# l646773422/h264-lab

Hardware: AMD Instinct MI355X
Metric: 1080p macroblocks/sec (higher is better)
Workload: dtype u8

## Files before the change

### h264-lab_amd/csrc/enc_mb.h

```cpp
#ifndef H264E_ENC_MB_H
#define H264E_ENC_MB_H

#include <stddef.h>
#include "enc_kernels.h"

struct GCtx { mv32 mv_left[4], mv_tl[4], mv_top[8]; };
#define GSCR_OFF(t) ((t) == 0 ? 0 : (t) == 1 ? 1024 : (t) == 2 ? 1536 : 2048)
#define GSCR_BYTES 2304

struct MbBuf
{
    alignas(16) uint8_t inp[256];
    alignas(16) uint8_t inp_c[128];
    alignas(16) uint8_t pred[256];
    alignas(4) uint8_t pix_top[36];
    alignas(4) uint8_t ptop[96];
    mv32 mv_top[8];
    uint8_t nnz_top[8];
    int8_t i4_top[4];
    uint32_t df_nz_top;
    int top_type, top_qp;
    mv32 mv[16], mvd[16];
    int type, cost, used_cand;
    mv32 mv_skip_pred;
};

struct RowLds
{
    mv32 mv_left[4], mv_tl[4];
    uint8_t nnz_left[8];
    int8_t i4_left[4];
    alignas(4) uint8_t pix_left[32];
    uint8_t pix_tl[4];
    uint32_t df_nzflag;
    mv32 df_mv[25];
    int left_type, left_qp;
    alignas(4) uint8_t strip_y[16*4];
    alignas(4) uint8_t strip_c[2][8*4];
    alignas(4) uint8_t brec[64];
    BitW bw;
    int skip_run, lead_skips, coded_any;
    int far_reads[3];
    int far_fail[3];
    int16_t slice_row[H264E_MAX_SLICES + 2];
    unsigned long long prof[4][32], prof_last[4], prof_c0, prof_w0;
    int f_noskip, f_bound, f_inter, f_decided, f_wdone, f_stop;
    int early_bound;
    int f_t3req, f_t3done;
    int f_front, d_type[2];
    int t3_sad_best, t3_lim[4];
    mv32 t3_mv_best;

    MbBuf mb[2];
    alignas(4) uint8_t trec[72];

    int8_t i4_mode[16];
    alignas(4) uint8_t bs[32];
    I4Scratch i4s;
    uint8_t nzctx[12];
    alignas(16) uint8_t pred_c[128];
    alignas(16) uint8_t i16pred[256];
    alignas(16) uint8_t tt[256];
    alignas(16) uint8_t i4rec[17*24];
    alignas(16) uint8_t ytile[20*YT_STRIDE];
    alignas(16) uint8_t ctile[2][10*CT_STRIDE];
    alignas(16) qblk_t qy[16];
    qblk_t qu[4], qv[4];
    int16_t dcy[16], dcu[4], dcv[4], lev_dcy[16], lev_dcu[4], lev_dcv[4];

    CavlcTab cavlc;
    DfTab dftab;
    int qconst[6];
    uint16_t qdat[2][42];

    mv32 part_mv[4][4], part_mvd[4][4];
    GCtx gctx[4];
    int gcost[4], gnum[4];
    alignas(16) uint8_t win[WIN_W*WIN_STRIDE + 16];
    alignas(16) uint8_t skip_pred[256];
    alignas(16) uint8_t skip_pred_c[128];
    alignas(16) uint8_t gtest[4][256];
    alignas(16) uint8_t gscr[GSCR_BYTES];

};
#define ROWLDS_INTRA_BYTES offsetof(RowLds, part_mv)

struct MbCtx
{
    const h264e_geom_t *G;
    int speed, slice_type;
    mv32 clu[2];
    const mv32 *clu_per_mb;
    Plane ref[3];
    RefView rv;
    gu8 *dec[3];
    int x, y, num, avail, type, cost, i16_mode, cropped, used_cand;
    int slice_top;
    mv32 mv_skip_pred;
    unsigned nz_mask;
    int qp;
    int lambda_mv, lambda_q4, skip_thr, skip_thr_i4, lambda_i4, lambda_i16;
};

struct rect_t { int x0, y0, x1, y1; };

DEV int in_rect(mv32 v, const rect_t &r) { return mvy(v) >= r.y0 && mvy(v) <= r.y1 && mvx(v) >= r.x0 && mvx(v) <= r.x1; }
DEV mv32 clip_rect(mv32 v, const rect_t &r) { return mvmk(imin(imax(mvx(v), r.x0), r.x1), imin(imax(mvy(v), r.y0), r.y1)); }
DEV mv32 mb_abs(const MbCtx &m, mv32 v) { return mvadd(v, mvmk(m.x*64, m.y*64)); }
DEV int mv_cost(const MbCtx &m, mv32 v, mv32 pred)
{
    return MUL_LAMBDA(se_len(mvx(v) - mvx(pred)) + se_len(mvy(v) - mvy(pred)), m.lambda_mv);
}
DEV rect_t mv_limit(const MbCtx &m) { rect_t r = { m.G->lim_x0, m.G->lim_y0, m.G->lim_x1, m.G->lim_y1 }; return r; }
DEV rect_t mv_qlimit(const MbCtx &m) { rect_t r = { m.G->lim_x0 + 16, m.G->lim_y0 + 16, m.G->lim_x1 - 16, m.G->lim_y1 - 16 }; return r; }


DEV int med3(int a, int b, int c) { return imax(imin(imax(a, b), c), imin(a, b)); }

DEV void mvp_put_arr(mv32 *mv_left, mv32 *mv_tl, mv32 *mv_top, int x, int y, int w, int h, mv32 mv)
{
    mv_tl[y] = mv_top[x + w - 1];
    for (int i = 1; i < h; i++) mv_tl[y + i] = mv;
    for (int i = 0; i < h; i++) mv_left[y + i] = mv;
    for (int i = 0; i < w; i++) mv_top[x + i] = mv;
}
DEV void mvp_put(RowLds &L, MbBuf &B, int x, int y, int w, int h, mv32 mv) { mvp_put_arr(L.mv_left, L.mv_tl, B.mv_top, x, y, w, h, mv); }

DEV mv32 mvp_get_arr(const mv32 *mv_left, const mv32 *mv_tl, const mv32 *mv_top, int flag, int x, int y, int w, int h)
{
    int type = 1;
    mv32 a = mv_left[y], b = mv_top[x], c = mv_top[x + w], d = mv_tl[y], ret = 0;
// ... 821 lines not shown
```

### h264-lab_amd/csrc/enc_row.h

```cpp
#ifndef H264E_ENC_ROW_H
#define H264E_ENC_ROW_H

#include "enc_mb.h"

#define GEOM_WIDE 0
#define GEOM_NARROW 1
#define GEOM_INTRA 2

struct ChainG
{
    GLOBAL_AS h264e_mbbottom_t *bottom;
    GLOBAL_AS h264e_mbpend_t *pend;
    GLOBAL_AS int *progress;
    GLOBAL_AS uint32_t *rowbits;
    GLOBAL_AS h264e_rowmeta_t *rowmeta;
    GLOBAL_AS h264e_mbrec_t *mbrec;
    GLOBAL_AS uint8_t *arena;
    uint32_t arena_cap;
    GLOBAL_AS uint8_t *nal_arena;
    uint32_t nal_cap;
    GLOBAL_AS uint32_t *cursor;
    GLOBAL_AS h264e_frameout_t *fout;
    GLOBAL_AS int *far_reads;
    unsigned long long *prof;
};
DEV ChainG chain_view(const h264e_chain_dev_t &C)
{
    ChainG g;
    g.bottom = (GLOBAL_AS h264e_mbbottom_t *)C.bottom; g.pend = (GLOBAL_AS h264e_mbpend_t *)C.pend; g.progress = (GLOBAL_AS int *)C.progress;
    g.rowbits = (GLOBAL_AS uint32_t *)C.rowbits; g.rowmeta = (GLOBAL_AS h264e_rowmeta_t *)C.rowmeta;
    g.mbrec = (GLOBAL_AS h264e_mbrec_t *)C.mbrec; g.arena = (GLOBAL_AS uint8_t *)C.arena; g.arena_cap = C.arena_cap; g.nal_arena = (GLOBAL_AS uint8_t *)C.nal_arena; g.nal_cap = C.nal_cap;
    g.cursor = (GLOBAL_AS uint32_t *)C.cursor; g.fout = (GLOBAL_AS h264e_frameout_t *)C.fout; g.far_reads = (GLOBAL_AS int *)C.far_reads; g.prof = C.prof;
    return g;
}

DEV void row_begin(RowLds &L, const h264e_geom_t &G, const ChainG &C, const h264e_frame_task_t &T, int row)
{
    WAVE_FOR(l)
    {
        if (l < 4) { L.mv_left[l] = 0; L.mv_tl[l] = 0; L.i4_left[l] = -1; L.pix_tl[l] = 0; }
        if (l < 8) L.nnz_left[l] = NNZ_NA;
        if (l < 32) L.pix_left[l] = 0;
        if (l < 25) L.df_mv[l] = 0;
        L.strip_y[l] = 0;
        L.strip_c[l >> 5][l & 31] = 0;
    }
    L.df_nzflag = 0;
    L.left_type = 0;
    L.left_qp = T.qp;
    L.bw.acc = 0; L.bw.nacc = 0; L.bw.pos = 0; L.bw.overflow = 0;
    L.bw.cap = (uint32_t)G.row_words;
    L.bw.buf = C.rowbits + (size_t)row*G.row_words;
    L.skip_run = 0; L.lead_skips = 0; L.coded_any = 0; L.far_reads[0] = L.far_reads[1] = L.far_reads[2] = 0; L.far_fail[0] = L.far_fail[1] = L.far_fail[2] = 0;
    L.f_noskip = L.f_bound = L.f_inter = L.f_decided = L.f_wdone = L.f_stop = 0; L.early_bound = 0; L.f_t3req = L.f_t3done = L.f_front = 0;
    WAVE_FOR(l) { if (l <= H264E_MAX_SLICES) L.slice_row[l] = l <= T.nslices ? T.slice_row[l] : (int16_t)0x7fff; }
    WAVE_FOR(l)
    {
        for (int k = l; k < 84; k += 64) L.qdat[k/42][k%42] = T.qdat[k/42][k%42];
    }
    cavlc_tab_load(L.cavlc);
    df_tab_load(L.dftab);
    L.qconst[0] = k_lambda_mv_q4[T.qp]; L.qconst[1] = k_lambda_q4[T.qp]; L.qconst[2] = k_skip_thr_inter[T.qp];
    L.qconst[3] = k_skip_thr_i4x4[T.qp]; L.qconst[4] = k_lambda_i4_q4[T.qp]; L.qconst[5] = k_lambda_i16_q4[T.qp];
    for (int i = 0; i < 32; i++) L.prof[0][i] = L.prof[1][i] = L.prof[2][i] = L.prof[3][i] = 0;
    L.prof_last[0] = L.prof_last[1] = 0;
    PROF_ROW_BEGIN(L);
    wave_sync();
    PROF_ROW_SYNC(L);
}

#define LOAD_TOP_ALL 0
#define LOAD_TOP_MV 1
#define LOAD_TOP_REST 2
template <int PART> DEV void load_top(RowLds &L, MbBuf &B, const h264e_geom_t &G, const GLOBAL_AS h264e_mbbottom_t *above, const GLOBAL_AS h264e_mbpend_t *pend_above, int x, int have_top)
{
    if (PART == LOAD_TOP_MV)
    {
        WAVE_FOR(l)
        {
            if (l < 4) B.mv_top[l] = have_top ? (mv32)cload32((const gu8 *)(above + x) + 32 + 4*l) : 0;
            else if (l == 4) B.mv_top[4] = (have_top && x + 1 < G.nmbx) ? (mv32)cload32((const gu8 *)(above + x + 1) + 32) : 0;
        }
        wave_sync();
        return;
    }
    if (have_top)
    {
        WAVE_FOR(l)
        {
            if (l < 16) lds32_store(L.trec + 4*l, cload32((const gu8 *)(above + x) + 4*l));
            else if (l == 16) lds32_store(L.trec + 64, x + 1 < G.nmbx ? cload32((const gu8 *)(above + x + 1)) : 0u);
            else if (l == 17) lds32_store(L.trec + 68, x + 1 < G.nmbx ? cload32((const gu8 *)(above + x + 1) + 32) : 0u);
            else if (l >= 32 && l < 56) lds32_store(B.ptop + 4*(l - 32), cload32((const gu8 *)(pend_above + x) + 4*(l - 32)));
        }
        wave_sync();
        WAVE_FOR(l)
        {
            if (l < 8) lds32_store(B.pix_top + 4*l, lds32(L.trec + 4*l));
            else if (l < 12) { if (PART == LOAD_TOP_ALL) B.mv_top[l - 8] = (mv32)lds32(L.trec + 32 + 4*(l - 8)); }
            else if (l < 20) B.nnz_top[l - 12] = L.trec[48 + l - 12];
            else if (l < 24) B.i4_top[l - 20] = (int8_t)L.trec[56 + l - 20];
            else if (l == 24) { B.df_nz_top = L.trec[60]; B.top_type = (int8_t)L.trec[61]; B.top_qp = L.trec[62]; }
            else if (l == 25) lds32_store(B.pix_top + 32, lds32(L.trec + 64));
            else if (l == 26) { if (PART == LOAD_TOP_ALL) B.mv_top[4] = (mv32)lds32(L.trec + 68); }
        }
    } else
    {
        WAVE_FOR(l)
        {
            if (l < 36) B.pix_top[l] = 0;
            if (l < 5 && PART == LOAD_TOP_ALL) B.mv_top[l] = 0;
            if (l < 8) B.nnz_top[l] = NNZ_NA;
            if (l < 4) B.i4_top[l] = -1;
            if (l == 0) { B.df_nz_top = 0; B.top_type = 0; B.top_qp = 0; }
        }
    }
    wave_sync();
}

DEV void load_input(MbBuf &B, const h264e_geom_t &G, const RowTask &T, int mbx, int mby)
{
    const bool inside = (mbx + 1)*16 <= G.width && (mby + 1)*16 <= G.height;
    WAVE_FOR(l)
    {
        {
            int r = l >> 2, c = l & 3, yy = imin(mby*16 + r, G.height - 1);
            const gu8 *p = (const gu8 *)T.in[0] + (size_t)yy*T.in_stride[0];
            uint32_t v = 0;
            if (inside) v = gload32(p + mbx*16 + 4*c);
            else for (int k = 0; k < 4; k++) v |= (uint32_t)p[imin(mbx*16 + 4*c + k, G.width - 1)] << (8*k);
            lds32_store(B.inp + 16*r + 4*c, v);
        }
        if (l < 32)
        {
            int pl = l >> 4, r = (l >> 1) & 7, c = l & 1, yy = imin(mby*8 + r, G.height/2 - 1);
            const gu8 *p = (const gu8 *)(pl ? T.in[2] : T.in[1]) + (size_t)yy*(pl ? T.in_stride[2] : T.in_stride[1]);
            uint32_t v = 0;
            if (inside) v = gload32(p + mbx*8 + 4*c);
            else for (int k = 0; k < 4; k++) v |= (uint32_t)p[imin(mbx*8 + 4*c + k, G.width/2 - 1)] << (8*k);
            lds32_store(B.inp_c + 16*r + 8*pl + 4*c, v);
        }
    }
    wave_sync();
}

template <int GEOM> DEV void row_prefetch(RowLds &L, const h264e_geom_t &G, const RowTask &T, int row, int x)
{
    load_input(L.mb[x & 1], G, T, x, row);
    if (GEOM != GEOM_INTRA && T.slice_type == 0)
    {
        Plane P;
        P.p = (const gu8 *)T.ref[0]; P.w = G.W; P.h = G.H; P.stride = G.W;
        wave_load_window(L.win, P, x*16 - WIN_M, row*16 - WIN_M, T.narrow);
    }
}

template <int GEOM> DEV void mb_ctx_init(MbCtx &m, RowLds &L, const h264e_geom_t &G, const RowTask &T, int row, int x, int row0, int side)
{
    const bool have_top = row > row0;
    m.G = &G;
    m.speed = T.speed; m.slice_type = T.slice_type; m.clu[0] = T.clusters[0]; m.clu[1] = T.clusters[1]; m.clu_per_mb = T.clusters_per_mb;
    for (int c = 0; c < 3; c++)
    {
        m.ref[c].p = (const gu8 *)T.ref[c];
        m.ref[c].w = G.W >> (c ? 1 : 0); m.ref[c].h = G.H >> (c ? 1 : 0); m.ref[c].stride = m.ref[c].w;
        m.dec[c] = (gu8 *)T.dec[c];
    }
    m.x = x; m.y = row; m.num = row*G.nmbx + x;
    m.avail = (have_top ? AV_T : 0) | (have_top && x != G.nmbx - 1 ? AV_TR : 0) | (x > 0 ? AV_L : 0) | (have_top && x > 0 ? AV_TL : 0);
    m.slice_top = !have_top;
    m.cropped = G.cropping && ((x + 1)*16 > G.width || (row + 1)*16 > G.height);
    m.type = 0; m.cost = 0x7FFFFFFF; m.i16_mode = 0; m.used_cand = 0; m.mv_skip_pred = 0; m.nz_mask = 0;
    m.qp = T.qp;
    m.lambda_mv = uni(L.qconst[0]); m.lambda_q4 = uni(L.qconst[1]); m.skip_thr = uni(L.qconst[2]);
    m.skip_thr_i4 = uni(L.qconst[3]); m.lambda_i4 = uni(L.qconst[4]); m.lambda_i16 = uni(L.qconst[5]);
    m.rv.dep = (const GLOBAL_AS int *)T.dep_progress; m.rv.nmbx = G.nmbx; m.rv.nmby = G.nmby;
    m.rv.P = m.ref[0]; m.rv.win = (const lu8 *)L.win; m.rv.has_win = GEOM != GEOM_INTRA && T.slice_type == 0; m.rv.wx0 = x*16 - WIN_M; m.rv.wy0 = row*16 - WIN_M;
    m.rv.vw = GEOM == GEOM_NARROW ? H264E_NARROW_VW : WIN_W; m.rv.vh = GEOM == GEOM_NARROW ? H264E_NARROW_VH : WIN_W; m.rv.far = &L.far_reads[side]; m.rv.fail = &L.far_fail[side]; m.rv.slice_row = L.slice_row; m.rv.nslices = T.nslices; m.rv.spin_limit = G.spin_limit;
}

struct NoSignals { DEVM void noskip() const {} DEVM void bound(int) const {} DEVM bool helper() const { return false; } DEVM void t3_request(mv32, int, const rect_t &) const {} DEVM bool t3_wait() const { return true; } };
template <int GEOM, class SIG> DEV void mb_search(RowLds &L, MbBuf &B, const h264e_geom_t &G, const RowTask &T, int row, int x, int row0, SIG sig)
{
    MbCtx m;
    mb_ctx_init<GEOM>(m, L, G, T, row, x, row0, 0);
    STAMP(L, 1);
    if (GEOM != GEOM_INTRA && T.slice_type == 0) inter_choose(L, B, m, sig);
    STAMP(L, 7);
    B.type = m.type; B.cost = m.cost; B.used_cand = m.used_cand; B.mv_skip_pred = m.mv_skip_pred;
    wave_sync();
}

struct InterIsThere
{
    DEVM bool ready() const { return true; }
    DEVM bool wait_noskip_or_ready() const { return true; }
    DEVM bool wait_bound_or_ready() const { return true; }
    DEVM bool wait_ready() const { return true; }
    DEVM int early_bound() const { return 0x7fffffff; }
    DEVM bool before_decide() const { return true; }
};

template <class P> DEV bool mb_intra_decide(RowLds &L, MbBuf &B, MbCtx &m, const RowTask &T, P pol)
{
    bool have = pol.ready();
    if (!have)
    {
        if (!pol.wait_noskip_or_ready()) return false;
        have = pol.ready();
// ... 584 lines not shown
```

### h264-lab_amd/csrc/h264e_dev.h

```cpp
#ifndef H264E_DEV_H
#define H264E_DEV_H
#include <stdint.h>

#define H264E_MV_NA 0x8000
#define H264E_ORDER_PAD 0xffffffffu
#define H264E_MAX_SLICES 16
#define H264E_ROW_BYTES_PER_MB 2048

#define H264E_DEP_ROWS 2
#define H264E_DEP_COLS 3
#define H264E_FRAME_LAG (2*H264E_DEP_ROWS + H264E_DEP_COLS)
#define H264E_NARROW_VW 53
#define H264E_NARROW_VH 52
#define H264E_NARROW_DEP_ROWS 1
#define H264E_NARROW_DEP_COLS 2
#define H264E_NARROW_FRAME_LAG (2*H264E_NARROW_DEP_ROWS + H264E_NARROW_DEP_COLS)

typedef int32_t mv32;

typedef struct
{
    int width, height;
    int W, H;
    int nmbx, nmby, nmb, cropping;
    int lim_x0, lim_y0, lim_x1, lim_y1;
    int row_words;
    unsigned spin_limit;
    int test_stall_row;
    int fz_wait_all;
} h264e_geom_t;

typedef struct
{
    uint8_t pix[32];
    mv32 mv[4];
    uint8_t nnz[8];
    int8_t i4[4];
    uint8_t df_nz;
    int8_t type;
    uint8_t qp;
    uint8_t pad;
} h264e_mbbottom_t;

typedef struct
{
    uint8_t y[64];
    uint8_t c[2][16];
} h264e_mbpend_t;

typedef struct
{
    uint32_t nbits;
    int32_t lead_skips;
    int32_t trail_skips;
    int32_t overflow;
} h264e_rowmeta_t;

typedef struct
{
    mv32 mv0;
    int8_t type;
    uint8_t used_cand;
    uint8_t pad[2];
} h264e_mbrec_t;

typedef struct
{
    uint32_t offset;
    uint32_t nbytes;
    int32_t nslices;
    uint32_t slice_nbytes[H264E_MAX_SLICES];
    int32_t all_skipped;
    int32_t clusters_moved;
    int32_t overflow;
    int32_t far_reads;
    int32_t pad[2];
} h264e_frameout_t;

#define H264E_WALK_OK 1
#define H264E_WALK_BAD 2
#define H264E_WALK_VOID 3
typedef struct
// ... 84 lines not shown
```

### h264-lab_amd/csrc/h264e_kernels.hip

```cpp
#include <stdio.h>
#include <stdlib.h>
#include <string.h>
#include "enc_row.h"
#include "enc_selftest.h"
#include "../../include/h264e_hip.h"

#include <hip/hip_runtime.h>





#ifndef H264E_POLL_SLEEP
#define H264E_POLL_SLEEP 16
#endif
DEV int poll_progress(const GLOBAL_AS int *flag, int need, int &seen, unsigned spin_limit)
{
    unsigned spins = 0;
    for (;;)
    {
        seen = uni(__hip_atomic_load(flag, __ATOMIC_RELAXED, __HIP_MEMORY_SCOPE_AGENT));
        if (seen >= need) return 0;
        if (seen < 0) return seen;
        if (++spins > spin_limit) return -1;
// ... 236 lines not shown
                for (int k = 0; k < H264E_MAX_SLICES; k++) hd->slice_nbytes[k] = nal_bytes[k];
                hd->clusters_moved = F.clusters_moved; hd->overflow = F.overflow | exp_overflow; hd->far_reads = F.far_reads;
                hd->walk_status = wstatus; hd->first_bad = first_bad; hd->state_out[0] = ws[0]; hd->state_out[1] = ws[1];
                __builtin_amdgcn_fence(__ATOMIC_RELEASE, "");
                asm volatile("s_waitcnt vmcnt(0)" ::: "memory");
                __hip_atomic_store(&hd->done, T.launch_id, __ATOMIC_RELAXED, __HIP_MEMORY_SCOPE_SYSTEM);
            }
        }
        FZ_STAMP(36);
#ifdef H264E_STAMPS
        if (LANE == 0 && C.prof) atomicAdd(C.prof + 37, 1ull);
#endif
        return;
    }

    if (row < T.first_row) return;
    if (job == 0 && row == G.test_stall_row) return;
    if (wv == 0) row_begin(L, G, C, T, row);
    if (WAVES >= 2) __syncthreads();
    const RowTask RT = rowtask_load(T);
    int row0 = 0, row1 = G.nmby;
    for (int k = 0; k < T.nslices; k++)
        if (row >= T.slice_row[k] && row < T.slice_row[k + 1]) { row0 = T.slice_row[k]; row1 = T.slice_row[k + 1]; }
    row0 = uni(row0); row1 = uni(row1);
    GLOBAL_AS int *my_progress = C.progress + row;
    GLOBAL_AS unsigned long long *mb_counter = (GLOBAL_AS unsigned long long *)uniptr(T.mb_counter);
    const auto count_mbs = [&](int n) { if (mb_counter && n > 0 && LANE == 0) __hip_atomic_fetch_add(mb_counter, (unsigned long long)n, __ATOMIC_RELAXED, __HIP_MEMORY_SCOPE_AGENT); };

    if (WAVES == 1 || wv == 0)
    {
        const GLOBAL_AS int *abort_word = (const GLOBAL_AS int *)uniptr(T.abort_word);
        const int launch_id = uni(T.launch_id);
        int seen = 0, seen_dep = 0;
        constexpr bool NARROW = GEOM == GEOM_NARROW;
        constexpr int DEP_ROWS = NARROW ? H264E_NARROW_DEP_ROWS : H264E_DEP_ROWS, DEP_COLS = NARROW ? H264E_NARROW_DEP_COLS : H264E_DEP_COLS;
        unsigned long long deps = 0;
        int ndeps = 0;
        if (T.dep_progress)
        {
            const int lo = imax(row - 2, 0), hi = imin(row + DEP_ROWS, G.nmby - 1);
            deps = (unsigned long long)hi; ndeps = 1;
            for (int k = T.nslices - 1; k >= 1; k--)
            {
                const int last = T.slice_row[k] - 1;
                if (last >= lo && last < hi) { deps |= (unsigned long long)last << (10*ndeps); ndeps++; }
            }
            ndeps = uni(ndeps);
        }
        for (int x = 0; x < G.nmbx; x++)
        {
            const int need = row > row0 ? imin(x + 2, G.nmbx) : 0;
            const int need_dep = RT.dep_progress ? imin(x + DEP_COLS, G.nmbx) : 0;
            int st = 0;
            const int abort_v = abort_word ? __hip_atomic_load(abort_word, __ATOMIC_RELAXED, __HIP_MEMORY_SCOPE_AGENT) : launch_id - 1;
            const GLOBAL_AS int *above = C.progress + (WAVES >= 2 ? G.nmby : 0) + (row - 1);
            const int early = seen < need ? __hip_atomic_load(above, __ATOMIC_RELAXED, __HIP_MEMORY_SCOPE_AGENT) : seen;
            if (seen_dep < need_dep)
            {
                int lowest = 0x7fffffff;
                for (int k = 0; k < ndeps && !st; k++)
                {
                    int sk = 0;
                    st = poll_progress((const GLOBAL_AS int *)RT.dep_progress + (int)((deps >> (10*k)) & 1023), need_dep, sk, G.spin_limit);
                    lowest = imin(lowest, sk);
                }
                seen_dep = lowest;
                if (!st) consumer_acquire();
            }
            STAMP(L, 13);
            if (WAVES >= 2 && !st && x >= 2) st = lds_wait(&L.f_wdone, x - 1, &L.f_stop);
            STAMP(L, 23);
            if (!st) row_prefetch<GEOM>(L, G, RT, row, x);
            STAMP(L, 0);
            if (uni(abort_v) == launch_id) st = -2;
            if (!st && seen < need)
            {
                seen = uni(early);
                if (seen < 0) st = seen;
                else if (seen < need) st = poll_progress(above, need, seen, G.spin_limit);
                if (!st) consumer_acquire();
            }
            STAMP(L, 13);
            if (!st) load_top<WAVES >= 2 ? LOAD_TOP_MV : LOAD_TOP_ALL>(L, L.mb[x & 1], G, C.bottom + (size_t)(row - 1)*G.nmbx, C.pend + (size_t)(row - 1)*G.nmbx, x, row > row0);
            STAMP(L, 0);
            if (WAVES >= 2 && !st && x >= 1) st = lds_wait(&L.f_decided, x, &L.f_stop);
            STAMP(L, 6);
            if (st)
            {
                if (WAVES >= 2) { flag_set(&L.f_stop, st); return; }
                if (LANE == 0)
                {
                    if (st == -1) *errflag = 1;
                    __hip_atomic_store(my_progress, st, __ATOMIC_RELAXED, __HIP_MEMORY_SCOPE_AGENT);
                }
                count_mbs(x);
                return;
            }
            if (WAVES == 1) row_step<GEOM>(L, G, C, RT, row, x, row0, row1);
            else mb_search<GEOM>(L, L.mb[x & 1], G, RT, row, x, row0, SearchSignals{ &L, x + 1, WAVES >= 3 });
            if (WAVES >= 3 && uni(flag_get(&L.f_stop))) return;
            {
                const int ff = uni(L.far_fail[0]) | (WAVES == 1 ? uni(L.far_fail[1]) : 0);
                if (ff)
                {
                    if (WAVES >= 2) { flag_set(&L.f_stop, ff < -2 ? -2 : ff); return; }
                    if (LANE == 0)
                    {
                        if (ff == -1) *errflag = 1;
                        __hip_atomic_store(my_progress, ff < -2 ? -2 : ff, __ATOMIC_RELAXED, __HIP_MEMORY_SCOPE_AGENT);
                    }
                    count_mbs(x);
                    return;
                }
            }
            if (WAVES >= 2) { flag_set(&L.f_inter, x + 1); STAMP(L, 14); continue; }
            asm volatile("s_waitcnt vmcnt(0)" ::: "memory");
            __builtin_amdgcn_wave_barrier();
            publish(my_progress, x + 1);
            STAMP(L, 14);
        }
        if (WAVES >= 2)
        {
#ifdef H264E_STAMPS
            if (LANE < 32 && C.prof) atomicAdd(C.prof + LANE, L.prof[0][LANE]);
#endif
            return;
        }
    } else if (WAVES >= 3 && wv == 2)
    {
        for (int x = 0; x < G.nmbx; x++)
        {
            int req = 0, st = 0;
            for (unsigned spins = 0;; spins++)
            {
                const int r3 = uni(flag_get(&L.f_t3req));
                if (r3 == x + 1) { req = 1; break; }
                if (r3 > x + 1) break;
                if (uni(flag_get(&L.f_inter)) >= x + 1) break;
                if (uni(flag_get(&L.f_stop))) { st = 1; break; }
                if (spins > LDS_SPIN_LIMIT) { flag_set(&L.f_stop, -1); st = 1; break; }
                __builtin_amdgcn_s_sleep(H264E_LDS_SLEEP);
            }
            if (st) return;
            if (!req) continue;
            MbCtx m;
            mb_ctx_init<GEOM>(m, L, G, RT, row, x, row0, 2);
            const rect_t lim = { uni(L.t3_lim[0]), uni(L.t3_lim[1]), uni(L.t3_lim[2]), uni(L.t3_lim[3]) };
            const mv32 mv_best = (mv32)uni(L.t3_mv_best);
            const int sad_best = uni(L.t3_sad_best);
            GRP_EACH(t)
            {
                if (t == 3) search_type(L, L.mb[x & 1], m, 3, mv_best, sad_best, lim, 0);
            }
            wave_sync();
            const int ff = uni(L.far_fail[2]);
            if (ff) { flag_set(&L.f_stop, ff < -2 ? -2 : ff); return; }
            flag_set(&L.f_t3done, x + 1);
        }
#ifdef H264E_STAMPS
        if (LANE < 32 && C.prof) atomicAdd(C.prof + LANE, L.prof[2][LANE]);
#endif
        return;
    } else if (WAVES == 4 && wv == 3)
    {
        for (int x = 0; x < G.nmbx; x++)
        {
            const int st = lds_wait(&L.f_front, x + 1, &L.f_stop);
            if (st)
            {
                if (LANE == 0) __hip_atomic_store(my_progress, st == -2 ? -2 : -1, __ATOMIC_RELAXED, __HIP_MEMORY_SCOPE_AGENT);
                return;
            }
            MbCtx m;
// ... 165 lines not shown
```

### h264-lab_amd/csrc/h264e_pool.h

```cpp
#ifndef H264E_POOL_H
#define H264E_POOL_H

static thread_local char g_err[256];
#define FAIL(...) do { snprintf(g_err, sizeof(g_err), __VA_ARGS__); return -1; } while (0)
extern "C" const char *h264e_hip_last_error(void) { return g_err; }


#define HIPCHK(x) do { hipError_t e_ = (x); if (e_ != hipSuccess) FAIL("%s: %s", #x, hipGetErrorString(e_)); } while (0)
static int dev_malloc(void **p, size_t n) { return hipMalloc(p, n ? n : 1) == hipSuccess ? 0 : -1; }
static void dev_free(void *p) { if (p) (void)hipFree(p); }

static int host_malloc(void **p, size_t n)
{
    if (hipHostMalloc(p, n ? n : 1, hipHostMallocMapped | hipHostMallocCoherent) != hipSuccess) return -1;
    memset(*p, 0, n ? n : 1);
    return 0;
}
static void host_free(void *p) { if (p) (void)hipHostFree(p); }

#define TASK_RING 128
static int imin_h(int a, int b) { return a < b ? a : b; }

#include <pthread.h>
#define H264E_MAX_DEVICES 64
// ... 221 lines not shown
        int *fill = (int *)calloc((size_t)8*jobs, sizeof(int));
        size_t cnt[8] = { 0 };
        if (!q || !fill) { free(q); free(fill); free(tmp); return -1; }
        for (size_t i = 0; i < 8*qlen; i++) q[i] = H264E_ORDER_PAD;
        int *want = (int *)calloc((size_t)8*jobs, sizeof(int));
        if (!want) { free(q); free(fill); free(tmp); return -1; }
        for (int i = 0; i < total; i++)
        {
            const int row = (int)(tmp[i] & 0xffffu), x = (row >= G.nmby ? bands - 1 : imin_h(bands - 1, row*bands/G.nmby)) & 7;
            want[8*(tmp[i] >> 16) + x]++;
        }
        int empty = 0;
        for (int i = 0; i < 8*jobs; i++) if (!want[i]) empty = 1;
        if (empty)
        {
            memcpy(ord, tmp, sizeof(uint32_t)*(size_t)total);
            free(q); free(fill); free(want); free(tmp);
            return 0;
        }
        for (int i = 0; i < total; i++)
        {
            const int row = (int)(tmp[i] & 0xffffu), jb = (int)(tmp[i] >> 16), x = (row >= G.nmby ? bands - 1 : imin_h(bands - 1, row*bands/G.nmby)) & 7;
            q[(size_t)x*qlen + cnt[x]++] = tmp[i];
            if (++fill[8*jb + x] == want[8*jb + x]) cnt[x] += (size_t)(per - want[8*jb + x]);
        }
        size_t n = 0;
        for (size_t k = 0; k < qlen; k++) for (int x = 0; x < 8; x++) ord[n++] = q[(size_t)x*qlen + k];
        p->order_count = n;
        free(q); free(fill); free(want); free(tmp);
    }
    return 0;
}

extern "C" int h264e_hip_pool_create(h264e_hip_pool_t **pool, int device, int width, int height, int nchains,
                                     int frames_resident, int slots)
{
    if (!pool || width <= 0 || height <= 0 || ((width | height) & 1) || nchains <= 0 || frames_resident <= 0 || slots <= 0)
        FAIL("h264e_hip_pool_create: bad argument");
    h264e_hip_pool_t *p = (h264e_hip_pool_t *)calloc(1, sizeof(*p));
    if (!p) FAIL("out of host memory");
    p->device = device; p->nchains = nchains; p->frames_resident = frames_resident; p->slots = slots;
    h264e_geom_t &G = p->G;
    G.width = width; G.height = height;
    G.nmbx = (width + 15) >> 4; G.nmby = (height + 15) >> 4; G.nmb = G.nmbx*G.nmby;
    G.W = G.nmbx*16; G.H = G.nmby*16;
    G.cropping = !!((width | height) & 15);
    G.lim_x0 = G.lim_y0 = -14*4;
    G.lim_x1 = (G.W - 2)*4; G.lim_y1 = (G.H - 2)*4;
    G.row_words = G.nmbx*(H264E_ROW_BYTES_PER_MB/4);
    const int knobs = getenv("H264E_TEST_KNOBS") && atoi(getenv("H264E_TEST_KNOBS")) == 1;
    G.spin_limit = 1u << 24;
    G.test_stall_row = -1;
    G.fz_wait_all = getenv("H264E_FZ_WAIT_ALL") ? atoi(getenv("H264E_FZ_WAIT_ALL")) : 0;
    p->test_upload_fail_at = -1;
    if (knobs)
    {
        if (getenv("H264E_TEST_ROW_BYTES_PER_MB")) { const int b = atoi(getenv("H264E_TEST_ROW_BYTES_PER_MB"))/4; G.row_words = G.nmbx*(b > 1 ? b : 1); }
        if (getenv("H264E_TEST_SPIN_LIMIT")) G.spin_limit = (unsigned)atol(getenv("H264E_TEST_SPIN_LIMIT"));
        if (getenv("H264E_TEST_STALL_ROW")) G.test_stall_row = atoi(getenv("H264E_TEST_STALL_ROW"));
        if (getenv("H264E_TEST_UPLOAD_FAIL_AT")) p->test_upload_fail_at = atoi(getenv("H264E_TEST_UPLOAD_FAIL_AT"));
    }
    p->frame_bytes = (size_t)width*height*3/2;
    p->waves = getenv("H264E_WAVES") ? atoi(getenv("H264E_WAVES")) : 0;
    if (p->waves != 1 && p->waves != 2 && p->waves != 3 && p->waves != 4) p->waves = 0;
    int ndev = 0;
    if (hipGetDeviceCount(&ndev) != hipSuccess || ndev <= 0)
    {
        free(p);
        FAIL("no HIP device: the HIP path is mandatory (there is no CPU fallback)");
    }
    if (hipSetDevice(device) != hipSuccess) { free(p); FAIL("hipSetDevice(%d) failed", device); }
    {
        const int share = getenv("H264E_SHARE_DEVICE") && atoi(getenv("H264E_SHARE_DEVICE")) == 1;
        if (process_guard_acquire(device)) { free(p); return -1; }
        p->guarded = !share;
    }
    if (hipStreamCreate(&p->stream) != hipSuccess || hipStreamCreate(&p->copy_stream) != hipSuccess || hipStreamCreate(&p->abort_stream) != hipSuccess) { if (p->guarded) process_guard_release(device); free(p); FAIL("hipStreamCreate failed"); }
    for (int i = 0; i < TASK_RING; i++) for (int k = 0; k < 3; k++) (void)hipEventCreate(&p->ev[i][k]);
    (void)hipEventCreate(&p->ev_t0); (void)hipEventCreate(&p->ev_t1); (void)hipEventCreate(&p->ev_prep);
    p->chains_host = (h264e_chain_dev_t *)calloc((size_t)nchains, sizeof(h264e_chain_dev_t));
    p->clu_dev = (int32_t **)calloc((size_t)nchains, sizeof(int32_t *));
    p->ref_sel = (int *)calloc((size_t)nchains, sizeof(int));
    p->traj_dev = (int32_t **)calloc((size_t)nchains, sizeof(int32_t *));
    p->traj_cur = (int *)calloc((size_t)nchains, sizeof(int));
    p->slot_launch = (int *)calloc((size_t)nchains, sizeof(int));
    p->host_rbsp = (uint8_t **)calloc((size_t)nchains, sizeof(uint8_t *));
    p->host_mbrec = (h264e_hip_mbrec_t **)calloc((size_t)nchains, sizeof(h264e_hip_mbrec_t *));
    int bad = 0;
    const size_t plane = (size_t)G.W*G.H*3/2;
    const uint32_t arena_cap = (uint32_t)((size_t)slots*((size_t)G.nmb*640 + 1024));
    const uint32_t nal_cap = (uint32_t)((size_t)G.nmb*660 + 4096);
    p->host_rbsp_cap = getenv("H264E_HOST_MIRROR_BYTES") ? (uint32_t)atol(getenv("H264E_HOST_MIRROR_BYTES")) : (uint32_t)((size_t)G.nmb*160 + 65536);
    if (p->host_rbsp_cap > nal_cap) p->host_rbsp_cap = nal_cap;
    for (int pass = 0; pass < 2 && !bad; pass++)
    {
        size_t pos = 0, hpos = 0;
        uint8_t *base = pass ? p->heap : 0, *hbase = pass ? p->hheap : 0;
        auto carve = [&](size_t n, size_t align) -> void * { pos = (pos + align - 1) & ~(align - 1); void *r = base ? base + pos : 0; pos += n ? n : 1; return r; };
        auto hcarve = [&](size_t n) -> void * { hpos = (hpos + 255) & ~(size_t)255; void *r = hbase ? hbase + hpos : 0; hpos += n; return r; };
        p->clip = (uint8_t *)carve(p->frame_bytes*(size_t)frames_resident, 4096);
        p->chains_dev = (h264e_chain_dev_t *)carve(sizeof(h264e_chain_dev_t)*(size_t)nchains, 256);
        p->tasks_dev = (h264e_frame_task_t *)carve(sizeof(h264e_frame_task_t)*(size_t)nchains*TASK_RING, 256);
        p->progress_all = (int *)carve(sizeof(int)*2*(size_t)nchains*G.nmby, 256);
        p->errflag = (int *)carve(sizeof(int), 256);
        p->mb_counter = (unsigned long long *)carve(sizeof(unsigned long long), 256);
        p->stepflags = (int *)carve(sizeof(int)*2*(size_t)nchains, 256);
// ... 901 lines not shown
```

### h264-lab_amd/csrc/wave.h

```cpp
#ifndef H264E_WAVE_H
#define H264E_WAVE_H

#include <stdint.h>
#include <string.h>

#ifdef H264E_EMU
extern "C" void emu_check_global(const void *p, size_t n, const char *file, int line);
#define EMU_GLOBAL(p, n) emu_check_global((const void *)(p), (n), __FILE__, __LINE__)
#define GLOBAL_AS
#define LDS_AS
#define NOINLINE_DEV static __attribute__((noinline))
#define DEV static inline
#define DEVM inline
#define DCONST static const
#ifdef H264E_EMU_REVERSE
#define WAVE_FOR(l) for (int l = 63; l >= 0; --l)
#else
#define WAVE_FOR(l) for (int l = 0; l < 64; ++l)
#endif
struct u32x4 { uint32_t x, y, z, w; };
DEV void wave_sync() {}
DEV int wave_lane() { return 0; }
DEV int uni(int v) { return v; }
template <class F> DEV int wave_sum(F f)
// ... 399 lines not shown
DEV uint64_t v64_nonzero_ballot(const V64 &a) { return __ballot(a.v != 0); }
#endif

#if defined(H264E_STAMPS) && !defined(H264E_EMU)
#define PROF_W ((int)(threadIdx.x >> 6))
#define STAMP(L, id) do { unsigned long long t_ = __builtin_readcyclecounter(); (L).prof[PROF_W][id] += t_ - (L).prof_last[PROF_W]; (L).prof_last[PROF_W] = t_; } while (0)
#define PCOUNT(L, id) do { (L).prof[PROF_W][id]++; } while (0)
#define PTIC() unsigned long long tic_ = __builtin_readcyclecounter()
#define PTOC(L, id) do { (L).prof[PROF_W][id] += __builtin_readcyclecounter() - tic_; } while (0)
#define PROF_ROW_BEGIN(L) do { (L).prof_c0 = __builtin_readcyclecounter(); (L).prof_w0 = wall_clock64(); } while (0)
#define PROF_ROW_SYNC(L) do { (L).prof_last[0] = (L).prof_last[1] = (L).prof_last[2] = (L).prof_last[3] = __builtin_readcyclecounter(); } while (0)
#define PROF_ROW_END(L, C) do { (L).prof[PROF_W][28] = __builtin_readcyclecounter() - (L).prof_c0; (L).prof[PROF_W][29] = wall_clock64() - (L).prof_w0; wave_sync(); \
                                if (LANE < 32 && (C).prof) atomicAdd((C).prof + LANE, (L).prof[PROF_W][LANE]); } while (0)
#else
#define STAMP(L, id) do { } while (0)
#define PCOUNT(L, id) do { } while (0)
#define PTIC() do { } while (0)
#define PTOC(L, id) do { } while (0)
#ifndef PROF_ROW_BEGIN
#define PROF_ROW_BEGIN(L) do { } while (0)
#define PROF_ROW_SYNC(L) do { } while (0)
#define PROF_ROW_END(L, C) do { } while (0)
#endif
#endif

struct LaneArr
{
#ifdef H264E_EMU
    int a[64];
    void clear() { for (int i = 0; i < 64; i++) a[i] = 0; }
    int get(int i) const { return a[i]; }
    void set(int i, int v) { a[i] = v; }
    int has(int v, int n) const { for (int i = 0; i < n; i++) if (a[i] == v) return 1; return 0; }
    int get_any(int i) const { return a[i & 63]; }
#else
    int r;
    __device__ __forceinline__ void clear() { r = 0; }
    __device__ __forceinline__ int get(int i) const { return __builtin_amdgcn_readlane(r, __builtin_amdgcn_readfirstlane(i)); }
    __device__ __forceinline__ void set(int i, int v) { r = (LANE == __builtin_amdgcn_readfirstlane(i)) ? __builtin_amdgcn_readfirstlane(v) : r; }
    __device__ __forceinline__ int has(int v, int n) const { return __ballot(LANE < n && r == __builtin_amdgcn_readfirstlane(v)) != 0; }
    __device__ __forceinline__ int get_any(int i) const { return __builtin_amdgcn_ds_bpermute(4*(i & 63), r); }
#endif
};

typedef LDS_AS uint8_t lu8;
typedef GLOBAL_AS uint8_t gu8;
typedef uint32_t __attribute__((aligned(1))) u32_unaligned;
typedef GLOBAL_AS u32_unaligned gu32u;

DEV uint32_t gload32(const gu8 *p) { EMU_GLOBAL(p, 4); return *(const gu32u *)p; }
DEV void gstore32(gu8 *p, uint32_t v) { EMU_GLOBAL(p, 4); *(gu32u *)p = v; }

#ifdef H264E_EMU
#define H264E_PLAIN_UNALIGNED_LOADS 0
DEV uint32_t cload32(const gu8 *p) { uint32_t v; EMU_GLOBAL(p, 4); memcpy(&v, p, 4); return v; }
DEV uint64_t cload64(const gu8 *p) { uint64_t v; EMU_GLOBAL(p, 8); memcpy(&v, p, 8); return v; }
DEV u32x4 cload128(const gu8 *p) { u32x4 v; EMU_GLOBAL(p, 16); memcpy(&v, p, 16); return v; }
DEV void cstore32(gu8 *p, uint32_t v) { EMU_GLOBAL(p, 4); memcpy(p, &v, 4); }
DEV void cstore64(gu8 *p, uint64_t v) { EMU_GLOBAL(p, 8); memcpy(p, &v, 8); }
#else
#ifndef H264E_COHERENT_LOADS
#define H264E_COHERENT_LOADS 0
#endif
#define H264E_PLAIN_UNALIGNED_LOADS (!H264E_COHERENT_LOADS)
#if H264E_COHERENT_LOADS
DEV uint32_t cload32(const gu8 *p) { return __hip_atomic_load((const GLOBAL_AS uint32_t *)p, __ATOMIC_RELAXED, __HIP_MEMORY_SCOPE_AGENT); }
DEV uint64_t cload64(const gu8 *p) { return __hip_atomic_load((const GLOBAL_AS uint64_t *)p, __ATOMIC_RELAXED, __HIP_MEMORY_SCOPE_AGENT); }
DEV void consumer_acquire() { __builtin_amdgcn_fence(__ATOMIC_ACQUIRE, "wavefront"); }
#else
DEV uint32_t cload32(const gu8 *p) { return *(const GLOBAL_AS uint32_t *)p; }
DEV uint64_t cload64(const gu8 *p) { return *(const GLOBAL_AS uint64_t *)p; }
DEV u32x4 cload128(const gu8 *p) { return *(const GLOBAL_AS u32x4 *)p; }
DEV void consumer_acquire()
{
    __builtin_amdgcn_fence(__ATOMIC_ACQUIRE, "agent");
    asm volatile("s_waitcnt vmcnt(0)" ::: "memory");
    __builtin_amdgcn_wave_barrier();
}
#endif
DEV void cstore32(gu8 *p, uint32_t v) { __hip_atomic_store((GLOBAL_AS uint32_t *)p, v, __ATOMIC_RELAXED, __HIP_MEMORY_SCOPE_AGENT); }
DEV void cstore64(gu8 *p, uint64_t v) { __hip_atomic_store((GLOBAL_AS uint64_t *)p, v, __ATOMIC_RELAXED, __HIP_MEMORY_SCOPE_AGENT); }
#endif

DEV int imin(int a, int b) { return a < b ? a : b; }
DEV int imax(int a, int b) { return a > b ? a : b; }
DEV int iabs(int x) { return x < 0 ? -x : x; }
DEV int clip255(int x) { return x < 0 ? 0 : x > 255 ? 255 : x; }
DEV int clip3(int lo, int hi, int x) { return x < lo ? lo : x > hi ? hi : x; }

#endif
```

Measured before the change: 13.69 million.

## Slide motion-search window and prefetch next macroblock via async LDS DMA

Instead of reloading the whole reference search window for every macroblock, the window is shifted left by 32 columns in LDS and only the new 32-column strip is fetched. The strip and the next macroblock's input pixels are loaded through global_load_lds DMA one macroblock ahead, so the loads overlap with the current macroblock's work. A look-ahead check of the dependency progress decides whether the next window can be staged early. The cost is extra LDS buffers, dma_wait calls on every exit path, and more complex prefetch-state bookkeeping that could cause stalls or hazards.

```diff
diff --git a/h264-lab_amd/csrc/enc_mb.h b/h264-lab_amd/csrc/enc_mb.h
--- a/h264-lab_amd/csrc/enc_mb.h
+++ b/h264-lab_amd/csrc/enc_mb.h
@@ -48,6 +48,10 @@
     int early_bound;
     int f_t3req, f_t3done;
     int f_front, d_type[2];
+    int pf;
+#ifdef H264E_STAMPS
+    unsigned prof_win[3];
+#endif
     int t3_sad_best, t3_lim[4];
     mv32 t3_mv_best;
 
@@ -77,6 +81,8 @@
     GCtx gctx[4];
     int gcost[4], gnum[4];
     alignas(16) uint8_t win[WIN_W*WIN_STRIDE + 16];
+    alignas(16) uint8_t win_next[WIN_W*32];
+    alignas(16) uint8_t inp_next[512];
     alignas(16) uint8_t skip_pred[256];
     alignas(16) uint8_t skip_pred_c[128];
     alignas(16) uint8_t gtest[4][256];
diff --git a/h264-lab_amd/csrc/enc_row.h b/h264-lab_amd/csrc/enc_row.h
--- a/h264-lab_amd/csrc/enc_row.h
+++ b/h264-lab_amd/csrc/enc_row.h
@@ -53,6 +53,10 @@
     L.bw.buf = C.rowbits + (size_t)row*G.row_words;
     L.skip_run = 0; L.lead_skips = 0; L.coded_any = 0; L.far_reads[0] = L.far_reads[1] = L.far_reads[2] = 0; L.far_fail[0] = L.far_fail[1] = L.far_fail[2] = 0;
     L.f_noskip = L.f_bound = L.f_inter = L.f_decided = L.f_wdone = L.f_stop = 0; L.early_bound = 0; L.f_t3req = L.f_t3done = L.f_front = 0;
+    L.pf = 0;
+#ifdef H264E_STAMPS
+    L.prof_win[0] = L.prof_win[1] = L.prof_win[2] = 0;
+#endif
     WAVE_FOR(l) { if (l <= H264E_MAX_SLICES) L.slice_row[l] = l <= T.nslices ? T.slice_row[l] : (int16_t)0x7fff; }
     WAVE_FOR(l)
     {
@@ -144,17 +148,91 @@
     wave_sync();
 }
 
-template <int GEOM> DEV void row_prefetch(RowLds &L, const h264e_geom_t &G, const RowTask &T, int row, int x)
-{
-    load_input(L.mb[x & 1], G, T, x, row);
-    if (GEOM != GEOM_INTRA && T.slice_type == 0)
-    {
-        Plane P;
-        P.p = (const gu8 *)T.ref[0]; P.w = G.W; P.h = G.H; P.stride = G.W;
-        wave_load_window(L.win, P, x*16 - WIN_M, row*16 - WIN_M, T.narrow);
-    }
-}
-
+DEV bool win_slides(const h264e_geom_t &G, int x) { return x >= 2 && x*16 - WIN_M + WIN_W <= G.W; }
+DEV void win_stage(RowLds &L, const Plane &P, int x, int row)
+{
+    const int wx0 = x*16 - WIN_M + 32, wy0 = row*16 - WIN_M;
+    for (int i = 0; i < 2; i++)
+        wave_dma<16>(L.win_next + 1024*i, [&](int l) -> const gu8 * {
+            const int s = 64*i + l, y = imin(imax(wy0 + (s >> 1), 0), P.h - 1);
+            return P.p + (size_t)y*P.stride + wx0 + 16*(s & 1);
+        });
+}
+DEV void win_slide(RowLds &L)
+{
+    WAVE_FOR(l)
+    {
+        uint8_t *d = L.win + l*WIN_STRIDE;
+        const uint8_t *n = L.win_next + 32*l;
+        uint32_t v[8];
+        for (int k = 0; k < 8; k++) v[k] = lds32(d + 16 + 4*k);
+        for (int k = 0; k < 8; k++) lds32_store(d + 4*k, v[k]);
+        for (int k = 0; k < 8; k++) v[k] = lds32(n + 4*k);
+        for (int k = 0; k < 8; k++) lds32_store(d + 32 + 4*k, v[k]);
+    }
+    wave_sync();
+}
+DEV bool inp_stageable(const RowTask &T)
+{
+    return (((uintptr_t)T.in[0] | (uintptr_t)T.in[1] | (uintptr_t)T.in[2] | (uintptr_t)(T.in_stride[0] | T.in_stride[1] | T.in_stride[2])) & 3) == 0;
+}
+DEV void inp_stage(RowLds &L, const RowTask &T, int mbx, int mby)
+{
+    wave_dma<4>(L.inp_next, [&](int l) -> const gu8 * {
+        return (const gu8 *)T.in[0] + (size_t)(mby*16 + (l >> 2))*T.in_stride[0] + mbx*16 + 4*(l & 3);
+    });
+    wave_dma<4>(L.inp_next + 256, [&](int l) -> const gu8 * {
+        const int r = (l >> 2) & 7, pl = (l >> 1) & 1;
+        return (const gu8 *)(pl ? T.in[2] : T.in[1]) + (size_t)(mby*8 + r)*(pl ? T.in_stride[2] : T.in_stride[1]) + mbx*8 + 4*(l & 1);
+    });
+}
+DEV void inp_from_stage(MbBuf &B, const RowLds &L)
+{
+    WAVE_FOR(l)
+    {
+        lds32_store(B.inp + 4*l, lds32(L.inp_next + 4*l));
+        if (l < 32) lds32_store(B.inp_c + 4*l, lds32(L.inp_next + 256 + 4*l));
+    }
+    wave_sync();
+}
+struct PrefetchAlways { DEVM bool operator()() const { return true; } };
+
+template <int GEOM, class PF = PrefetchAlways> DEV void row_prefetch(RowLds &L, const h264e_geom_t &G, const RowTask &T, int row, int x, PF next_ok = PF())
+{
+    const bool inter = GEOM != GEOM_INTRA && T.slice_type == 0;
+    const bool slide = GEOM != GEOM_INTRA && G.win_slide;
+    Plane P;
+    P.p = (const gu8 *)T.ref[0]; P.w = G.W; P.h = G.H; P.stride = G.W;
+    const int pf = slide ? uni(L.pf) : 0;
+    const bool pf_inp = pf == 4*(x + 1) + 1 || pf == 4*(x + 1) + 3, pf_win = pf >= 4*(x + 1) + 2 && pf <= 4*(x + 1) + 3;
+    if (pf_inp) inp_from_stage(L.mb[x & 1], L);
+    else load_input(L.mb[x & 1], G, T, x, row);
+    if (inter)
+    {
+        if (slide && win_slides(G, x))
+        {
+            if (!pf_win) { win_stage(L, P, x, row); dma_wait(); }
+            win_slide(L);
+#ifdef H264E_STAMPS
+            if (LANE == 0) L.prof_win[pf_win ? 0 : 1]++;
+#endif
+        } else
+        {
+            wave_load_window(L.win, P, x*16 - WIN_M, row*16 - WIN_M, T.narrow);
+#ifdef H264E_STAMPS
+            if (LANE == 0) L.prof_win[2]++;
+#endif
+        }
+    }
+    if (slide && x + 1 < G.nmbx)
+    {
+        const bool inp = (x + 2)*16 <= G.width && (row + 1)*16 <= G.height && inp_stageable(T);
+        const bool win = inter && win_slides(G, x + 1) && next_ok();
+        if (inp) inp_stage(L, T, x + 1, row);
+        if (win) win_stage(L, P, x + 1, row);
+        L.pf = 4*(x + 2) + (inp ? 1 : 0) + (win ? 2 : 0);
+    }
+}
 template <int GEOM> DEV void mb_ctx_init(MbCtx &m, RowLds &L, const h264e_geom_t &G, const RowTask &T, int row, int x, int row0, int side)
 {
     const bool have_top = row > row0;
diff --git a/h264-lab_amd/csrc/h264e_dev.h b/h264-lab_amd/csrc/h264e_dev.h
--- a/h264-lab_amd/csrc/h264e_dev.h
+++ b/h264-lab_amd/csrc/h264e_dev.h
@@ -28,6 +28,7 @@
     unsigned spin_limit;
     int test_stall_row;
     int fz_wait_all;
+    int win_slide;
 } h264e_geom_t;
 
 typedef struct
diff --git a/h264-lab_amd/csrc/h264e_kernels.hip b/h264-lab_amd/csrc/h264e_kernels.hip
--- a/h264-lab_amd/csrc/h264e_kernels.hip
+++ b/h264-lab_amd/csrc/h264e_kernels.hip
@@ -312,6 +312,7 @@
             const int need = row > row0 ? imin(x + 2, G.nmbx) : 0;
             const int need_dep = RT.dep_progress ? imin(x + DEP_COLS, G.nmbx) : 0;
             int st = 0;
+            dma_wait();
             const int abort_v = abort_word ? __hip_atomic_load(abort_word, __ATOMIC_RELAXED, __HIP_MEMORY_SCOPE_AGENT) : launch_id - 1;
             const GLOBAL_AS int *above = C.progress + (WAVES >= 2 ? G.nmby : 0) + (row - 1);
             const int early = seen < need ? __hip_atomic_load(above, __ATOMIC_RELAXED, __HIP_MEMORY_SCOPE_AGENT) : seen;
@@ -330,7 +331,18 @@
             STAMP(L, 13);
             if (WAVES >= 2 && !st && x >= 2) st = lds_wait(&L.f_wdone, x - 1, &L.f_stop);
             STAMP(L, 23);
-            if (!st) row_prefetch<GEOM>(L, G, RT, row, x);
+            const int need_dep1 = RT.dep_progress ? imin(x + 1 + DEP_COLS, G.nmbx) : 0;
+            const bool look = !st && G.win_slide && seen_dep < need_dep1 && ndeps == 1 && x + 1 < G.nmbx;
+            const int look0 = look ? __hip_atomic_load((const GLOBAL_AS int *)RT.dep_progress + (int)(deps & 1023), __ATOMIC_RELAXED, __HIP_MEMORY_SCOPE_AGENT) : 0;
+            if (!st) row_prefetch<GEOM>(L, G, RT, row, x, [&]() -> bool {
+                if (seen_dep >= need_dep1) return true;
+                if (!look) return false;
+                const int lk = uni(look0);
+                if (lk < need_dep1) return false;
+                consumer_acquire();
+                seen_dep = lk;
+                return true;
+            });
             STAMP(L, 0);
             if (uni(abort_v) == launch_id) st = -2;
             if (!st && seen < need)
@@ -347,6 +359,7 @@
             STAMP(L, 6);
             if (st)
             {
+                dma_wait();
                 if (WAVES >= 2) { flag_set(&L.f_stop, st); return; }
                 if (LANE == 0)
                 {
@@ -358,11 +371,12 @@
             }
             if (WAVES == 1) row_step<GEOM>(L, G, C, RT, row, x, row0, row1);
             else mb_search<GEOM>(L, L.mb[x & 1], G, RT, row, x, row0, SearchSignals{ &L, x + 1, WAVES >= 3 });
-            if (WAVES >= 3 && uni(flag_get(&L.f_stop))) return;
+            if (WAVES >= 3 && uni(flag_get(&L.f_stop))) { dma_wait(); return; }
             {
                 const int ff = uni(L.far_fail[0]) | (WAVES == 1 ? uni(L.far_fail[1]) : 0);
                 if (ff)
                 {
+                    dma_wait();
                     if (WAVES >= 2) { flag_set(&L.f_stop, ff < -2 ? -2 : ff); return; }
                     if (LANE == 0)
                     {
@@ -379,6 +393,10 @@
             publish(my_progress, x + 1);
             STAMP(L, 14);
         }
+        dma_wait();
+#ifdef H264E_STAMPS
+        if (LANE < 3 && C.prof) atomicAdd(C.prof + 40 + LANE, (unsigned long long)L.prof_win[LANE]);
+#endif
         if (WAVES >= 2)
         {
 #ifdef H264E_STAMPS
diff --git a/h264-lab_amd/csrc/h264e_pool.h b/h264-lab_amd/csrc/h264e_pool.h
--- a/h264-lab_amd/csrc/h264e_pool.h
+++ b/h264-lab_amd/csrc/h264e_pool.h
@@ -297,6 +297,7 @@
     G.spin_limit = 1u << 24;
     G.test_stall_row = -1;
     G.fz_wait_all = getenv("H264E_FZ_WAIT_ALL") ? atoi(getenv("H264E_FZ_WAIT_ALL")) : 0;
+    G.win_slide = getenv("H264E_WIN_SLIDE") ? atoi(getenv("H264E_WIN_SLIDE")) != 0 : 1;
     p->test_upload_fail_at = -1;
     if (knobs)
     {
diff --git a/h264-lab_amd/csrc/wave.h b/h264-lab_amd/csrc/wave.h
--- a/h264-lab_amd/csrc/wave.h
+++ b/h264-lab_amd/csrc/wave.h
@@ -475,6 +475,24 @@
 DEV void gstore32(gu8 *p, uint32_t v) { EMU_GLOBAL(p, 4); *(gu32u *)p = v; }
 
 #ifdef H264E_EMU
+template <int N, class F> DEV void wave_dma(uint8_t *lds, F src)
+{
+    static_assert(N == 4 || N == 16, "LDS-DMA widths used here: 4, 16 bytes");
+    WAVE_FOR(l) { const gu8 *s = src(l); EMU_GLOBAL(s, N); memcpy(lds + N*l, s, N); }
+}
+DEV void dma_wait() {}
+#else
+template <int N, class F> DEV void wave_dma(uint8_t *lds, F src)
+{
+    static_assert(N == 4 || N == 16, "LDS-DMA widths used here: 4, 16 bytes");
+    const GLOBAL_AS void *s = (const GLOBAL_AS void *)src(LANE);
+    if constexpr (N == 16) __builtin_amdgcn_global_load_lds(s, (LDS_AS void *)lds, 16, 0, 0);
+    else __builtin_amdgcn_global_load_lds(s, (LDS_AS void *)lds, 4, 0, 0);
+}
+DEV void dma_wait() { asm volatile("s_waitcnt vmcnt(0)" ::: "memory"); __builtin_amdgcn_wave_barrier(); }
+#endif
+
+#ifdef H264E_EMU
 #define H264E_PLAIN_UNALIGNED_LOADS 0
 DEV uint32_t cload32(const gu8 *p) { uint32_t v; EMU_GLOBAL(p, 4); memcpy(&v, p, 4); return v; }
 DEV uint64_t cload64(const gu8 *p) { uint64_t v; EMU_GLOBAL(p, 8); memcpy(&v, p, 8); return v; }
```

Result: no change. 13.68 million, median of 3 (-0.1%).
